# SMLC-NYSBC/TARGET-VAE

Hardware: AMD Instinct MI355X
Metric: training images/sec (fwd+bwd+Adam), P8 z=2 64x64 bs=256/GPU (higher is better)
Workload: dtype f32 (matrix products: operands as TWO fp16 parts under one power-of-two scale PER ROW of the operand (row / column of the product), 3 fp16 MFMAs per product block -- 2 where one operand is the exact 0 / 1 matrix -- fp32 accumulate: at least as accurate against fp64 as the fp32 matrix pipe (profiles/

## Files before the change

target-vae_amd/csrc/dense_wgrad_x6_instance.hip:

```cpp
#include "abi_dense_x6.hpp"

using namespace tvae;

#define TVAE_WG_ONE(V_, X_, L_, NP_)                                                                                  \
    do {                                                                                                              \
        hipError_t e_ = allow_big_lds(dense_wgrad_x6_dma_kernel<V_, X_, L_, NP_>, WG_RING_BYTES);                     \
        if (e_ != hipSuccess) return (int)e_;                                                                         \
        hipLaunchKernelGGL((dense_wgrad_x6_dma_kernel<V_, X_, L_, NP_>), dim3(tm.grid()), dim3(DX6_THREADS),           \
                           WG_RING_BYTES, st, dY, ldd, X, ldx, ws, M, Kf, N, nchunk, tm, bt, dy_stride, vg, va, atile, hs); \
        return (int)hipGetLastError();                                                                                \
    } while (0)
#define TVAE_WG_LAUNCH_DEF(NP_)                                                                                       \
    namespace tvae {                                                                                                  \
    int dense_wgrad_x6_launch_p##NP_(TVAE_WG_LAUNCH_ARGS) {                                                           \
        switch (variant) {                                                                                            \
            case 0: TVAE_WG_ONE(false, false, 0, NP_);                                                            \
            case 1: TVAE_WG_ONE(true, false, 0, NP_);                                                             \
            case 2: TVAE_WG_ONE(false, true, 0, NP_);                                                             \
            case 3: TVAE_WG_ONE(true, true, 0, NP_);                                                              \
            case 5: TVAE_WG_ONE(true, false, 1, NP_);                                                                 \
            case 7: TVAE_WG_ONE(true, true, 1, NP_);                                                                  \
            case 9: TVAE_WG_ONE(true, false, 2, NP_);                                                                 \
            case 11: TVAE_WG_ONE(true, true, 2, NP_);                                                                 \
            default: return (int)hipErrorInvalidValue;                                                                \
        }                                                                                                             \
    }                                                                                                                 \
    }

#define TVAE_WG_LAUNCH_DEF_ABF                                                                                        \
    namespace tvae {                                                                                                  \
    int dense_wgrad_x6_launch_p1_abf(TVAE_WG_LAUNCH_ARGS) {                                                           \
        if (variant != 0) return (int)hipErrorInvalidValue;                                                           \
        hipError_t e_ = allow_big_lds(dense_wgrad_x6_dma_kernel<false, false, 0, 1, true>, WG_RING_BYTES);            \
        if (e_ != hipSuccess) return (int)e_;                                                                         \
        hipLaunchKernelGGL((dense_wgrad_x6_dma_kernel<false, false, 0, 1, true>), dim3(tm.grid()), dim3(DX6_THREADS),  \
                           WG_RING_BYTES, st, dY, ldd, X, ldx, ws, M, Kf, N, nchunk, tm, bt, dy_stride, vg, va, atile, hs); \
        return (int)hipGetLastError();                                                                                \
    }                                                                                                                 \
    }

#define TVAE_WGW_LAUNCH_DEF(NP_)                                                                                      \
    namespace tvae {                                                                                                  \
    int dense_wgrad_x6_wide_p##NP_(TVAE_WGW_LAUNCH_ARGS) {                                                            \
        if (M % WW_ROWS != 0 || Kf <= 128 || bt.tiles_per_batch <= 0 ||                                             \
            tm.tilesN != (Kf <= 160 ? 1 : cdiv(Kf, 192)))                                                             \
            return (int)hipErrorInvalidValue;                                                                         \
        const unsigned grid_ =                                                                                        \
            8u * cdiv(tm.splits * (tm.tilesM / bt.tiles_per_batch), 8) * bt.tiles_per_batch * tm.tilesN;              \
        if (Kf <= 160) {              \
            hipError_t e_ = allow_big_lds(dense_wgrad_x6_wide_kernel<NP_, 5>, WW_RING_BYTES);                         \
            if (e_ != hipSuccess) return (int)e_;                                                                     \
            hipLaunchKernelGGL((dense_wgrad_x6_wide_kernel<NP_, 5>), dim3(grid_), dim3(DX6_THREADS), WW_RING_BYTES, st, \
                               dY, ldd, X, ldx, ws, M, Kf, N, nchunk, tm, bt, dy_stride, atile, hs);                  \
            return (int)hipGetLastError();                                                                            \
        }                                                                                                             \
        hipError_t e_ = allow_big_lds(dense_wgrad_x6_wide_kernel<NP_, 6>, WW_RING_BYTES);                             \
        if (e_ != hipSuccess) return (int)e_;                                                                         \
        hipLaunchKernelGGL((dense_wgrad_x6_wide_kernel<NP_, 6>), dim3(grid_), dim3(DX6_THREADS), WW_RING_BYTES, st,   \
                           dY, ldd, X, ldx, ws, M, Kf, N, nchunk, tm, bt, dy_stride, atile, hs);                      \
        return (int)hipGetLastError();                                                                                \
    }                                                                                                                 \
    }

#if TVAE_WG_NP == 1
TVAE_WG_LAUNCH_DEF(1)
TVAE_WG_LAUNCH_DEF_ABF
#elif TVAE_WG_NP == 2
TVAE_WG_LAUNCH_DEF(2)
TVAE_WGW_LAUNCH_DEF(2)
#elif TVAE_WG_NP == 3
TVAE_WG_LAUNCH_DEF(3)
TVAE_WGW_LAUNCH_DEF(3)
#else
#error "dense_wgrad_x6_instance.hip is compiled once per number of parts: -DTVAE_WG_NP=1, 2 or 3"
#endif
```

target-vae_amd/csrc/dense_x6_kernels.hpp:

```cpp
#pragma once
#include <hip/hip_runtime.h>
#include <type_traits>
#include "conv_x6_device.hpp"
#include "small_device.hpp"

#ifndef TVAE_ABL
#define TVAE_ABL 0
#endif

namespace tvae {

template <int NP>
__device__ __forceinline__ void mfma_np(f32x16& acc, const Cell16 (&a)[3], const Cell16 (&b)[3]) {
    if (NP == 3) mfma6(acc, a, b);
    else if (NP == 2) mfma3h(acc, a, b);
    else acc = __builtin_amdgcn_mfma_f32_32x32x16_bf16(a[0].v, b[0].v, acc, 0, 0, 0);
}
template <int NP>
__device__ __forceinline__ void mfma_part(f32x16& acc, const Cell16& a, const Cell16& b) {
    if (NP == 2) acc = __builtin_amdgcn_mfma_f32_32x32x16_f16(a.h, b.h, acc, 0, 0, 0);
    else acc = __builtin_amdgcn_mfma_f32_32x32x16_bf16(a.v, b.v, acc, 0, 0, 0);
}
template <int NP> struct OneBits { static constexpr unsigned lo = NP == 2 ? 0x3c00u : 0x3f80u, hi = lo << 16; };
template <bool XS>
// ... 753 lines not shown
    if (!tm.decode(blockIdx.x, tile_m, tile_n, split_unused)) return;
    int batch = 0;
    if (bt.tiles_per_batch > 0) {
        batch = tile_m / bt.tiles_per_batch;
        X += batch * bt.x_stride;
        ep.C += batch * bt.c_stride;
    }
    const int m0g = tile_m * DX4_ROWS;
    const int m0 = m0g - batch * bt.tiles_per_batch * DX4_ROWS, n0 = tile_n * 128;
    const int khalf = lane >> 5;
    const int nk = K8pad >> 1;
    bsm[tid] = (ep.bias && (m0 + tid) < M) ? ep.bias[(m0 + tid) >> ep.bias_shift] : 0.f;
    __shared__ __attribute__((aligned(16))) float h3a_[NP == 2 ? DX4_ROWS : 4];
    __shared__ float h3x_[NP == 2 ? 128 : 1];
    float sx = 1.f;
    if (NP == 2) {
        h3a_[tid] = h3_inv(h3_scale(hs.amax_a[hs.a_rows ? m0g + tid : 0]));
        if (hs.x_group > 0) sx = h3_scale(hs.amax_x[(long)batch * hs.x_bstride + min((n0 + (tid & 127)) / hs.x_group, hs.x_bstride - 1)]);
        else sx = h3_scale(hs.amax_x[0]);
        if (tid < 128) h3x_[tid] = h3_inv(sx);
    }

    const long part_cells = (long)K8pad * Mpad;
    const uint4* a_ptr = A3 + (long)khalf * Mpad + m0g + 64 * wave + (lane & 31);
    auto load_a = [&](int t, Cell16 (&a)[2][3]) {
        const uint4* q = a_ptr + (long)(2 * t) * Mpad;
#pragma unroll
        for (int i = 0; i < 2; ++i)
#pragma unroll
            for (int p = 0; p < NP; ++p) a[i][p].u = q[p * part_cells + i * 32];
    };
    const int kq = tid >> 7, nb = tid & 127;
    const float* x_col = X + n0 + nb;
    auto load_x = [&](int t, float (&x)[2][4]) {
#pragma unroll
        for (int h = 0; h < 2; ++h) {
            const int kb = 16 * t + 4 * (kq + 2 * h);
#pragma unroll
            for (int j = 0; j < 4; ++j) x[h][j] = x_col[(long)min(kb + j, K - 1) * ldx];
        }
    };
    auto store_b = [&](int stage, const float (&x)[2][4]) {
#pragma unroll
        for (int h = 0; h < 2; ++h) {
            uint2* dst = reinterpret_cast<uint2*>(Bs + stage * 768 + h * 128 + nb) + kq;
            if (NP == 1) {
                dst[0] = make_uint2(bf16_pair(x[h][0], x[h][1]), bf16_pair(x[h][2], x[h][3]));
                continue;
            }
            if (NP == 2) {
                unsigned hw[2], lw[2];
#pragma unroll
                for (int q = 0; q < 2; ++q) split2h_pair(x[h][2 * q] * sx, x[h][2 * q + 1] * sx, hw[q], lw[q]);
                dst[0] = make_uint2(hw[0], hw[1]);
                dst[2 * 256] = make_uint2(lw[0], lw[1]);
                continue;
            }
            unsigned hw[2], mw[2], lw[2];
#pragma unroll
            for (int q = 0; q < 2; ++q) split3_pair(x[h][2 * q], x[h][2 * q + 1], hw[q], mw[q], lw[q]);
            dst[0] = make_uint2(hw[0], hw[1]);
            dst[2 * 256] = make_uint2(mw[0], mw[1]);
            dst[2 * 512] = make_uint2(lw[0], lw[1]);
        }
    };
    f32x16 acc[2][4];
#pragma unroll
    for (int i = 0; i < 2; ++i)
#pragma unroll
        for (int j = 0; j < 4; ++j)
#pragma unroll
            for (int r = 0; r < 16; ++r) acc[i][j][r] = 0.f;
    Cell16 afA[2][3], afB[2][3];
    float xA[2][4], xB[2][4];
    {
        float x0[2][4];
        load_x(0, x0);
        load_a(0, afA);
        load_x(nk > 1 ? 1 : 0, xB);
        load_x(nk > 2 ? 2 : 0, xA);
        store_b(0, x0);
    }
    __syncthreads();
    auto step = [&](int t, Cell16 (&afc)[2][3], Cell16 (&afn)[2][3], float (&xn)[2][4]) {
        const int cur = t & 1;
        load_a(t + 1 < nk ? t + 1 : t, afn);
        const uint4* bs = Bs + cur * 768 + khalf * 128 + (lane & 31);
#pragma unroll
        for (int j = 0; j < 4; ++j) {
            Cell16 bf[3];
#pragma unroll
            for (int p = 0; p < NP; ++p) bf[p].u = bs[p * 256 + j * 32];
            mfma_np<NP>(acc[0][j], afc[0], bf);
            mfma_np<NP>(acc[1][j], afc[1], bf);
            if (j == 1) {
                store_b(cur ^ 1, xn);
                load_x(t + 3 < nk ? t + 3 : t, xn);
            }
        }
        __builtin_amdgcn_sched_barrier(0);
        __syncthreads();
    };
    int tt = 0;
    for (; tt + 1 < nk; tt += 2) {
        step(tt, afA, afB, xB);
        step(tt + 1, afB, afA, xA);
    }
    if (nk & 1) step(nk - 1, afA, afB, xB);
    if (EPI == 1) {
        if (m0 < M) dense_x6_epilogue_store<NP>(acc, ep.C, ep.ldc, (long)tile_n * ep.ctile, h3a_, h3x_, wave, lane, m0);
        return;
    }
    if (EPI == 2) {
        unsigned short* c16 = reinterpret_cast<unsigned short*>(ep.C - (long)batch * bt.c_stride) + (long)batch * bt.c_stride;
        if (m0 < M) dense_x6_epilogue_store_bf16(acc, c16, ep.ldc, (long)tile_n * ep.ctile, wave, lane, m0);
        return;
    }
    if (NP == 2) h3_unscale_rc<true>(acc, h3a_, h3x_, wave, lane);
    float ysum[4] = {0.f, 0.f, 0.f, 0.f};
    float gsum[4][2] = {{0.f, 0.f}, {0.f, 0.f}, {0.f, 0.f}, {0.f, 0.f}};
    const float gyv[4] = {0.f, 0.f, 0.f, 0.f};
    const InTail it{nullptr, nullptr, nullptr, nullptr, nullptr, nullptr, 1};
    float vmax_ = 0.f;
    if (TVAE_ABL & 8) {
        float t_ = 0.f;
#pragma unroll
        for (int i = 0; i < 2; ++i)
#pragma unroll
            for (int j = 0; j < 4; ++j)
#pragma unroll
                for (int r = 0; r < 16; ++r) t_ += acc[i][j][r];
        if (t_ == 123.456f) ep.C[0] = t_;
    } else
    if (ep.act == ACT_LRELU)
        dense_x6_epilogue<ACT_LRELU, ACT_NONE, false, false, false>(acc, ep, bsm, m0, n0, M, wave, lane, nullptr, ysum, it, nullptr,
                                                                     gsum, tile_n, nullptr, gyv, 0.f, nullptr, 0, vmax_);
    else if (ep.act == ACT_TANH)
        dense_x6_epilogue<ACT_TANH, ACT_NONE, false, false, false>(acc, ep, bsm, m0, n0, M, wave, lane, nullptr, ysum, it, nullptr,
                                                                    gsum, tile_n, nullptr, gyv, 0.f, nullptr, 0, vmax_);
    else
        dense_x6_epilogue<ACT_NONE, ACT_NONE, false, false, false>(acc, ep, bsm, m0, n0, M, wave, lane, nullptr, ysum, it, nullptr,
                                                                    gsum, tile_n, nullptr, gyv, 0.f, nullptr, 0, vmax_);
}

struct ATile {
    int sh;
    int mask;
    long ts;
};
constexpr ATile ATILE_PLAIN = {30, 0x3fffffff, 0};

constexpr int WG_SLOT_BYTES = 4096 + 1024 + 256;
constexpr int WG_RING_BYTES = 8 * 3 * WG_SLOT_BYTES;

template <bool VIRT, bool XVA, int LRF, int NP, bool ABF = false>
static __global__ __launch_bounds__(DX6_THREADS, 2)
void dense_wgrad_x6_dma_kernel(const float* __restrict__ dY, long ldd, const float* __restrict__ X, long ldx, float* ws,
                               int M, int Kf, int N, int nchunk, TileMap tm, DenseBatch bt, long dy_stride, VirtGrad vg,
                               VirtAct va, ATile atile, H3Scale hs) {
    static_assert(!ABF || (NP == 1 && !VIRT && !XVA && LRF == 0), "bf16-stored A: one-part mode, plain operands");
    constexpr int NDMA = (ABF ? 2 : (LRF == 2 ? 2 : 4)) + (XVA ? 2 : 1) + (VIRT ? 1 : 0);
    __shared__ __attribute__((aligned(16))) uint4 Bs[2 * 3 * 2 * 128];
    extern __shared__ __attribute__((aligned(16))) unsigned char wg_ring[];
    const int tid = threadIdx.x, lane = tid & 63;
    const int wave = __builtin_amdgcn_readfirstlane(tid >> 6);
    int tile_m, tile_k, split;
    if (!tm.decode(blockIdx.x, tile_m, tile_k, split)) return;
    int batch = 0, nbatch = 1;
    if (bt.tiles_per_batch > 0) {
        batch = tile_m / bt.tiles_per_batch;
        nbatch = tm.tilesM / bt.tiles_per_batch;
        tile_m -= batch * bt.tiles_per_batch;
        dY += (ABF ? batch * dy_stride / 2 : batch * dy_stride);
        X += batch * bt.x_stride;
    }
    const int m0 = tile_m * DX6_ROWS, k0 = tile_k * 128;
    const int nbeg = split * nchunk;
    const int nend = min(N, nbeg + nchunk);
    const int nk = (nend - nbeg) >> 4;
    const int khalf = lane >> 5;
    if (nk <= 0) {
#pragma unroll
        for (int i = 0; i < 2; ++i)
#pragma unroll
            for (int r = 0; r < 16; ++r) {
                const int m = m0 + wave * 64 + i * 32 + (r & 3) + 8 * (r >> 2) + 4 * khalf;
                if (m >= M) continue;
                float* wrow = ws + (((long)split * nbatch + batch) * M + m) * Kf + k0 + (lane & 31);
#pragma unroll
                for (int j = 0; j < 4; ++j)
                    if (k0 + j * 32 + (lane & 31) < Kf) wrow[j * 32] = 0.f;
            }
        return;
    }

    auto a_scale_of = [&](int m) -> float {
        return h3_scale(hs.amax_a[hs.a_rows ? (long)batch * hs.a_bstride + (hs.a_mod > 0 ? m % hs.a_mod : m) : 0]);
    };
    float sa[2] = {1.f, 1.f};
    if (NP == 2 && !LRF) {
#pragma unroll
        for (int i = 0; i < 2; ++i) sa[i] = a_scale_of(min(m0 + 64 * wave + 32 * i + (lane & 31), M - 1));
    }
    const float* d_ptr[4];
#pragma unroll
    for (int g = 0; g < 4; ++g) {
        if (ABF) {
            const int row = m0 + 64 * wave + 32 * (g & 1) + (lane & 31);
            d_ptr[g] = reinterpret_cast<const float*>(reinterpret_cast<const unsigned short*>(dY) +
                                                      (long)min(row, M - 1) * ldd + 8 * (lane >> 5));
        } else {
            const int row = m0 + 64 * wave + 16 * g + (lane >> 2);
            d_ptr[g] = dY + (long)min(row, M - 1) * ldd + 4 * ((lane & 3) ^ ((lane >> 4) & 3));
        }
    }
    const unsigned* b_ptr[2] = {nullptr, nullptr};
    if (LRF == 2) {
#pragma unroll
        for (int i = 0; i < 2; ++i)
            b_ptr[i] = vg.bits + (long)min(m0 + 64 * wave + 32 * i + (lane & 31), M - 1) * (N >> 5);
    }
    const int kr = tid >> 2, q4 = tid & 3;
    const int kx = min(k0 + kr, Kf - 1);
    const float b_ok = (k0 + kr) < Kf ? 1.f : 0.f;
    const float* x_src = XVA ? va.xr + 2 * (long)nbeg + (lane & 31) : X + (long)kx * ldx + nbeg + 4 * q4;
    const float* lb_src = XVA ? (va.lb ? va.lb + kx : va.bc + kx) : nullptr;
    const float lb_on = (XVA && va.lb) ? 1.f : 0.f;
    const float* g_src = VIRT ? vg.gy + nbeg + (lane & 15) : nullptr;
    const float va_w0 = XVA ? va.wc[2 * kx] : 0.f, va_w1 = XVA ? va.wc[2 * kx + 1] : 0.f, va_bc = XVA ? va.bc[kx] : 0.f;
    float sx = 1.f;
    if (NP == 2) {
        if (XVA && LRF) sx = h3_scale(__fmaf_rn(fabsf(va_w0) + fabsf(va_w1), hs.amax_x[0], hs.amax_x[4 + kx]) * hs.amax_x[3]);
        else if (hs.x_group > 0) sx = h3_scale(hs.amax_x[(long)batch * hs.x_bstride + kx / hs.x_group]);
        else sx = h3_scale(hs.amax_x[0]);
    }
    const unsigned ring_lds = (unsigned)(size_t)(__attribute__((address_space(3))) void*)wg_ring +
                              (unsigned)(wave * 3 * WG_SLOT_BYTES);
    const unsigned char* ring = wg_ring + wave * 3 * WG_SLOT_BYTES;
    auto dma_step = [&](int slot, int t) {
        const int na = nbeg + 16 * t;
        const long off = (long)(na >> atile.sh) * atile.ts + (na & atile.mask);
        const unsigned sl = ring_lds + (unsigned)(slot * WG_SLOT_BYTES);
        if (ABF) {
#pragma unroll
            for (int g = 0; g < 2; ++g) {
                const unsigned short* src = reinterpret_cast<const unsigned short*>(d_ptr[g]) + off;
                const unsigned dst = sl + (unsigned)(g * 1024);
                asm volatile("s_mov_b32 m0, %0\n\ts_nop 0\n\tglobal_load_lds_dwordx4 %1, off" :: "s"(dst), "v"(src) : "memory", "m0");
            }
        } else if (LRF == 2) {
#pragma unroll
            for (int i = 0; i < 2; ++i) {
                const unsigned* src = b_ptr[i] + (na >> 5);
                const unsigned dst = sl + (unsigned)(i * 256);
                asm volatile("s_mov_b32 m0, %0\n\ts_nop 0\n\tglobal_load_lds_dword %1, off" :: "s"(dst), "v"(src) : "memory", "m0");
            }
        } else {
#pragma unroll
            for (int g = 0; g < 4; ++g) {
                const float* src = d_ptr[g] + off;
                const unsigned dst = sl + (unsigned)(g * 1024);
                asm volatile("s_mov_b32 m0, %0\n\ts_nop 0\n\tglobal_load_lds_dwordx4 %1, off" :: "s"(dst), "v"(src) : "memory", "m0");
            }
        }
        if (XVA) {
            const float* sx = x_src + 32 * t;
            const unsigned dx = sl + 4096u;
            asm volatile("s_mov_b32 m0, %0\n\ts_nop 0\n\tglobal_load_lds_dword %1, off" :: "s"(dx), "v"(sx) : "memory", "m0");
            const float* slb = lb_src + (long)(lb_on != 0.f ? na / va.Np : 0) * Kf;
            const unsigned dl = sl + 4096u + 256u;
            asm volatile("s_mov_b32 m0, %0\n\ts_nop 0\n\tglobal_load_lds_dword %1, off" :: "s"(dl), "v"(slb) : "memory", "m0");
        } else {
            const float* sx = x_src + 16 * t;
            const unsigned dx = sl + 4096u;
            asm volatile("s_mov_b32 m0, %0\n\ts_nop 0\n\tglobal_load_lds_dwordx4 %1, off" :: "s"(dx), "v"(sx) : "memory", "m0");
        }
        if (VIRT) {
            const float* sg = g_src + 16 * t;
            const unsigned dg = sl + 4096u + 1024u;
            asm volatile("s_mov_b32 m0, %0\n\ts_nop 0\n\tglobal_load_lds_dword %1, off" :: "s"(dg), "v"(sg) : "memory", "m0");
        }
    };
    int a_at[2][2];
#pragma unroll
    for (int i = 0; i < 2; ++i)
#pragma unroll
        for (int h = 0; h < 2; ++h)
            a_at[i][h] = (2 * i + ((lane >> 4) & 1)) * 1024 + (lane & 15) * 64 + (((2 * khalf + h) ^ ((lane >> 2) & 3)) * 16);
    auto read_a = [&](int slot, float4 (&r)[2][2], float4 (&gq)[2]) {
        const unsigned char* sl = ring + slot * WG_SLOT_BYTES;
        if (ABF) {
#pragma unroll
            for (int i = 0; i < 2; ++i) r[i][0] = *reinterpret_cast<const float4*>(sl + i * 1024 + 16 * lane);
            return;
        }
        if (LRF == 2) {
#pragma unroll
            for (int i = 0; i < 2; ++i) r[i][0].x = *reinterpret_cast<const float*>(sl + i * 256 + 4 * lane);
            return;
        }
#pragma unroll
        for (int i = 0; i < 2; ++i)
#pragma unroll
            for (int h = 0; h < 2; ++h) r[i][h] = *reinterpret_cast<const float4*>(sl + a_at[i][h]);
        if (VIRT && !LRF) {
            gq[0] = *reinterpret_cast<const float4*>(sl + 4096 + 1024 + 32 * khalf);
            gq[1] = *reinterpret_cast<const float4*>(sl + 4096 + 1024 + 32 * khalf + 16);
        }
    };
    const bool xva_lrelu = XVA && va.act == ACT_LRELU;
    auto read_x = [&](int slot) -> float4 {
        const unsigned char* sl = ring + slot * WG_SLOT_BYTES + 4096;
        if (XVA) {
            const float4 c0 = *reinterpret_cast<const float4*>(sl + 32 * q4);
            const float4 c1 = *reinterpret_cast<const float4*>(sl + 32 * q4 + 16);
            const float lbv = *reinterpret_cast<const float*>(sl + 256 + 4 * lane) * lb_on;
            if (xva_lrelu) {
                const float p0 = dec_l0_pre(va_w0, va_w1, va_bc, lbv, c0.x, c0.y), p1 = dec_l0_pre(va_w0, va_w1, va_bc, lbv, c0.z, c0.w);
                const float p2 = dec_l0_pre(va_w0, va_w1, va_bc, lbv, c1.x, c1.y), p3 = dec_l0_pre(va_w0, va_w1, va_bc, lbv, c1.z, c1.w);
                if (va.slope > 0.f && va.slope < 1.f)
                    return make_float4(fmaxf(p0, p0 * va.slope), fmaxf(p1, p1 * va.slope), fmaxf(p2, p2 * va.slope),
                                       fmaxf(p3, p3 * va.slope));
                return make_float4(p0 > 0.f ? p0 : p0 * va.slope, p1 > 0.f ? p1 : p1 * va.slope, p2 > 0.f ? p2 : p2 * va.slope,
                                   p3 > 0.f ? p3 : p3 * va.slope);
            }
            return make_float4(act_apply(dec_l0_pre(va_w0, va_w1, va_bc, lbv, c0.x, c0.y), va.act, va.slope),
                               act_apply(dec_l0_pre(va_w0, va_w1, va_bc, lbv, c0.z, c0.w), va.act, va.slope),
                               act_apply(dec_l0_pre(va_w0, va_w1, va_bc, lbv, c1.x, c1.y), va.act, va.slope),
                               act_apply(dec_l0_pre(va_w0, va_w1, va_bc, lbv, c1.z, c1.w), va.act, va.slope));
        }
        return *reinterpret_cast<const float4*>(sl + 16 * lane);
    };
    float a_ok[2];
#pragma unroll
    for (int i = 0; i < 2; ++i) {
        const int m = m0 + 64 * wave + 32 * i + (lane & 31);
        a_ok[i] = m < M ? ((VIRT && !LRF) ? vg.wo[m] : 1.f) : 0.f;
    }
    auto virt_a = [&](float4 (&r)[2][2], const float4 (&gq)[2]) {
        if (VIRT && !LRF) {
#pragma unroll
            for (int i = 0; i < 2; ++i)
#pragma unroll
                for (int h = 0; h < 2; ++h)
                    r[i][h] = make_float4(virt_value(vg, r[i][h].x, 1.f, gq[h].x), virt_value(vg, r[i][h].y, 1.f, gq[h].y),
                                          virt_value(vg, r[i][h].z, 1.f, gq[h].z), virt_value(vg, r[i][h].w, 1.f, gq[h].w));
        }
    };
    auto split_a = [&](const float4 (&r)[2][2], Cell16 (&a)[2][3], int t) {
        if (ABF) {
#pragma unroll
            for (int i = 0; i < 2; ++i)
                a[i][0].u = make_uint4(__float_as_uint(r[i][0].x), __float_as_uint(r[i][0].y), __float_as_uint(r[i][0].z),
                                       __float_as_uint(r[i][0].w));
            return;
        }
        if (LRF == 2) {
            const int sh = ((nbeg + 16 * t) & 31) + 8 * khalf;
#pragma unroll
            for (int i = 0; i < 2; ++i) {
                const unsigned b = (__float_as_uint(r[i][0].x) >> sh) & 0xffu;
                const unsigned y = b | (b << 15);
#pragma unroll
                for (int q = 0; q < 4; ++q) a[i][0].w[q] = (y & (0x00010001u << (2 * q))) * (OneBits<NP>::lo >> (2 * q));
            }
            return;
        }
        if (LRF) {
#pragma unroll
            for (int i = 0; i < 2; ++i) {
                const float v[8] = {r[i][0].x, r[i][0].y, r[i][0].z, r[i][0].w, r[i][1].x, r[i][1].y, r[i][1].z, r[i][1].w};
#pragma unroll
                for (int q = 0; q < 4; ++q)
                    a[i][0].w[q] = (v[2 * q] > 0.f ? OneBits<NP>::lo : 0u) | (v[2 * q + 1] > 0.f ? OneBits<NP>::hi : 0u);
            }
            return;
        }
#pragma unroll
        for (int i = 0; i < 2; ++i) {
            const float f = NP == 2 ? a_ok[i] * sa[i] : a_ok[i];
            const float v[8] = {r[i][0].x * f, r[i][0].y * f, r[i][0].z * f, r[i][0].w * f,
                                r[i][1].x * f, r[i][1].y * f, r[i][1].z * f, r[i][1].w * f};
            if (NP == 1) {
#pragma unroll
                for (int q = 0; q < 4; ++q) a[i][0].w[q] = bf16_pair(v[2 * q], v[2 * q + 1]);
            } else if (NP == 2) {
                split2hx8(v, a[i][0], a[i][1]);
            } else {
                split3x8(v, a[i][0], a[i][1], a[i][2]);
            }
        }
    };
    float ssum = 0.f;
    const float bsx = NP == 2 ? b_ok * sx : b_ok;
    auto store_b = [&](int stage, const float4& x, int slot, bool real_step) {
        unsigned hw[2], mw[2], lw[2];
        float4 gm = make_float4(bsx, bsx, bsx, bsx);
        if (LRF) {
            const float4 g4 = *reinterpret_cast<const float4*>(ring + slot * WG_SLOT_BYTES + 4096 + 1024 + 16 * q4);
            gm = make_float4(g4.x * bsx, g4.y * bsx, g4.z * bsx, g4.w * bsx);
        }
        const float v[4] = {x.x * gm.x, x.y * gm.y, x.z * gm.z, x.w * gm.w};
        if (LRF && real_step) ssum += (v[0] + v[1]) + (v[2] + v[3]);
        uint2* dst = reinterpret_cast<uint2*>(Bs + stage * 768 + (q4 >> 1) * 128 + kr) + (q4 & 1);
        if (NP == 1) {
            dst[0] = make_uint2(bf16_pair(v[0], v[1]), bf16_pair(v[2], v[3]));
            return;
        }
        if (NP == 2) {
#pragma unroll
            for (int q = 0; q < 2; ++q) split2h_pair(v[2 * q], v[2 * q + 1], hw[q], lw[q]);
            dst[0] = make_uint2(hw[0], hw[1]);
            dst[2 * 256] = make_uint2(lw[0], lw[1]);
            return;
        }
#pragma unroll
        for (int q = 0; q < 2; ++q) split3_pair(v[2 * q], v[2 * q + 1], hw[q], mw[q], lw[q]);
        dst[0] = make_uint2(hw[0], hw[1]);
        dst[2 * 256] = make_uint2(mw[0], mw[1]);
        dst[2 * 512] = make_uint2(lw[0], lw[1]);
    };

    f32x16 acc[2][4];
#pragma unroll
    for (int i = 0; i < 2; ++i)
#pragma unroll
        for (int j = 0; j < 4; ++j)
#pragma unroll
            for (int r = 0; r < 16; ++r) acc[i][j][r] = 0.f;

    Cell16 af[2][3];
    const int tl = nk - 1;
    {
        dma_step(0, 0);
        dma_step(1, min(1, tl));
        dma_step(2, min(2, tl));
        asm volatile("s_waitcnt vmcnt(%0)" :: "n"(2 * NDMA) : "memory");
        float4 ar[2][2], g0[2];
        read_a(0, ar, g0);
        virt_a(ar, g0);
        split_a(ar, af, 0);
        store_b(0, read_x(0), 0, true);
    }
    __syncthreads();
    int s_next = 1, s_dma = 0;
    for (int t = 0; t < nk; ++t) {
        const int cur = t & 1;
        asm volatile("s_waitcnt vmcnt(%0)" :: "n"(NDMA) : "memory");
        dma_step(s_dma, min(t + 3, tl));
        Cell16 an[2][3];
        const uint4* bs = Bs + cur * 768 + khalf * 128 + (lane & 31);
#pragma unroll
        for (int j = 0; j < 4; ++j) {
            Cell16 bf[3];
#pragma unroll
            for (int p = 0; p < NP; ++p) bf[p].u = bs[p * 256 + j * 32];
            if (LRF) {
#pragma unroll
                for (int i = 0; i < 2; ++i)
#pragma unroll
                    for (int p = 0; p < NP; ++p) mfma_part<NP>(acc[i][j], af[i][0], bf[p]);
            } else {
                mfma_np<NP>(acc[0][j], af[0], bf);
                mfma_np<NP>(acc[1][j], af[1], bf);
            }
            if (j == 0) {
                float4 ar[2][2], gn[2];
                read_a(s_next, ar, gn);
                virt_a(ar, gn);
                split_a(ar, an, min(t + 1, tl));
            }
            if (j == 1) store_b(cur ^ 1, read_x(s_next), s_next, t + 1 < nk);
        }
#pragma unroll
        for (int i = 0; i < 2; ++i)
#pragma unroll
            for (int p = 0; p < 3; ++p) af[i][p] = an[i][p];
        s_next = s_next == 2 ? 0 : s_next + 1;
        s_dma = s_dma == 2 ? 0 : s_dma + 1;
        __builtin_amdgcn_sched_barrier(0);
        __syncthreads();
    }
    asm volatile("s_waitcnt vmcnt(0)" ::: "memory");
    float sk[4] = {0.f, 0.f, 0.f, 0.f};
    float ixv[4] = {1.f, 1.f, 1.f, 1.f};
    float* ssm = reinterpret_cast<float*>(Bs);
    if (LRF) {
        ssum += __shfl_xor(ssum, 1, 64);
        ssum += __shfl_xor(ssum, 2, 64);
        if (q4 == 0) ssm[kr] = NP == 2 ? ssum * h3_inv(sx) : ssum;
    }
    if (NP == 2) {
        if (q4 == 0) ssm[128 + kr] = h3_inv(sx);
        if (!LRF) ssm[256 + tid] = h3_inv(a_scale_of(min(m0 + tid, M - 1)));
    }
    if (LRF || NP == 2) __syncthreads();
    if (LRF) {
#pragma unroll
        for (int j = 0; j < 4; ++j) sk[j] = vg.slope * ssm[j * 32 + (lane & 31)];
    }
    if (NP == 2) {
#pragma unroll
        for (int j = 0; j < 4; ++j) ixv[j] = ssm[128 + j * 32 + (lane & 31)];
    }
    const float oms = 1.f - vg.slope;
    if (TVAE_ABL & 8) {
        float t_ = 0.f;
#pragma unroll
        for (int i = 0; i < 2; ++i)
#pragma unroll
            for (int j = 0; j < 4; ++j)
#pragma unroll
                for (int r = 0; r < 16; ++r) t_ += acc[i][j][r];
        if (t_ == 123.456f) ws[0] = t_;
        return;
    }
#pragma unroll
    for (int i = 0; i < 2; ++i)
#pragma unroll
        for (int r = 0; r < 16; ++r) {
            const int rl = wave * 64 + i * 32 + (r & 3) + 8 * (r >> 2) + 4 * (lane >> 5);
            const int m = m0 + rl;
            if (m >= M) continue;
            const float wm = (LRF && !vg.raw) ? vg.wo[m] : 1.f;
            const float ia = (NP == 2 && !LRF) ? ssm[256 + rl] : 1.f;
            float* wrow = ws + (((long)split * nbatch + batch) * M + m) * Kf + k0 + (lane & 31);
#pragma unroll
            for (int j = 0; j < 4; ++j)
                if (k0 + j * 32 + (lane & 31) < Kf) {
                    const float a = NP == 2 ? (acc[i][j][r] * ia) * ixv[j] : acc[i][j][r];
                    wrow[j * 32] = LRF ? wm * __fmaf_rn(oms, a, sk[j]) : a;
                }
        }
}

template <int NP, int NK>
static __global__ __launch_bounds__(256, 1)
void dense_x6_xres_kernel(const uint4* __restrict__ A3, const float* __restrict__ X, long ldx, float* __restrict__ C, long ldc,
                           long ctile, int M, int Mb, int Mpad, int K, int nprob, int tilesN, int nch, long x_stride,
                           long c_stride, H3Scale hs) {
    extern __shared__ __attribute__((aligned(16))) unsigned char xres_lds[];
    const int tid = threadIdx.x, lane = tid & 63;
    const int wave = __builtin_amdgcn_readfirstlane(tid >> 6);
    constexpr int K8pad = 2 * NK;
    uint4* Bs = reinterpret_cast<uint4*>(xres_lds);
    float* h3a_ = reinterpret_cast<float*>(xres_lds + (size_t)NK * NP * 256 * 16);
    float* h3x_ = h3a_ + Mb;
    const int cs = (tilesN + nch - 1) / nch;
    const int g = ((blockIdx.x >> 3) / cs) * 8 + (blockIdx.x & 7), r = (blockIdx.x >> 3) % cs;
    const int batch = g / nch, tile_n = (g - batch * nch) * cs + r;
    if (batch >= nprob || tile_n >= tilesN) return;
    X += batch * x_stride;
    C += batch * c_stride + (long)tile_n * ctile;
    const int n0 = tile_n * 128;
    const int khalf = lane >> 5;
    {
        const int kq = tid >> 7, nb = tid & 127;
        float sx = 1.f;
        if (NP == 2) {
            sx = hs.x_group > 0 ? h3_scale(hs.amax_x[(long)batch * hs.x_bstride + min((n0 + nb) / hs.x_group, hs.x_bstride - 1)])
                                : h3_scale(hs.amax_x[0]);
            if (tid < 128) h3x_[tid] = h3_inv(sx);
            for (int m = tid; m < Mb; m += 256) h3a_[m] = h3_inv(h3_scale(hs.amax_a[hs.a_rows ? batch * Mb + m : 0]));
        }
        const float* x_col = X + n0 + nb;
#pragma unroll
        for (int t0 = 0; t0 < NK; t0 += 3) {
            float x[3][2][4];
#pragma unroll
            for (int u = 0; u < 3; ++u)
#pragma unroll
                for (int h = 0; h < 2; ++h)
#pragma unroll
                    for (int j = 0; j < 4; ++j) {
                        const int k = 16 * (t0 + u < NK ? t0 + u : NK - 1) + 4 * (kq + 2 * h) + j;
                        x[u][h][j] = x_col[(long)min(k, K - 1) * ldx];
                    }
#pragma unroll
            for (int u = 0; u < 3; ++u) {
                if (t0 + u >= NK) break;
#pragma unroll
                for (int h = 0; h < 2; ++h) {
                    uint2* dst = reinterpret_cast<uint2*>(Bs + (size_t)(t0 + u) * NP * 256 + h * 128 + nb) + kq;
                    if (NP == 2) {
                        unsigned hw[2], lw[2];
#pragma unroll
                        for (int q = 0; q < 2; ++q) split2h_pair(x[u][h][2 * q] * sx, x[u][h][2 * q + 1] * sx, hw[q], lw[q]);
                        dst[0] = make_uint2(hw[0], hw[1]);
                        dst[2 * 256] = make_uint2(lw[0], lw[1]);
                    } else {
                        unsigned hw[2], mw[2], lw[2];
#pragma unroll
                        for (int q = 0; q < 2; ++q) split3_pair(x[u][h][2 * q], x[u][h][2 * q + 1], hw[q], mw[q], lw[q]);
                        dst[0] = make_uint2(hw[0], hw[1]);
                        dst[2 * 256] = make_uint2(mw[0], mw[1]);
                        dst[2 * 512] = make_uint2(lw[0], lw[1]);
                    }
                }
            }
        }
    }
    __syncthreads();
    const long part_cells = (long)K8pad * Mpad;
    const uint4* bs0 = Bs + khalf * 128 + (lane & 31);
    const uint4* a_base = A3 + (long)khalf * Mpad + (long)batch * Mb + (lane & 31);
    float ixv[4];
#pragma unroll
    for (int j = 0; j < 4; ++j) ixv[j] = NP == 2 ? h3x_[j * 32 + (lane & 31)] : 1.f;
    const unsigned loff = (unsigned)((4 * khalf * ldc + (lane & 31)) * 4);
    auto store_row = [&](const f32x16 (&acc)[2][4], int mp, int s_) {
        const int i = s_ >> 4, q = (s_ >> 2) & 3, p = s_ & 3;
        const int row = mp + 32 * i + 8 * q + p;
        float* rowp = reinterpret_cast<float*>(reinterpret_cast<char*>(C + (long)row * ldc) + loff);
        const float ia = NP == 2 ? h3a_[row + 4 * khalf] : 1.f;
#pragma unroll
        for (int j = 0; j < 4; ++j) {
            const float v = NP == 2 ? (acc[i][j][4 * q + p] * ixv[j]) * ia : acc[i][j][4 * q + p];
            __builtin_nontemporal_store(v, rowp + j * 32);
        }
    };
    auto block = [&](f32x16 (&accC)[2][4], int mc, const f32x16 (&accP)[2][4], int mp, bool have_prev) {
        const uint4* a_run[NP];
#pragma unroll
        for (int p = 0; p < NP; ++p) a_run[p] = a_base + mc + p * part_cells;
#ifndef TVAE_XRES2_NB
#define TVAE_XRES2_NB 8
#endif
        constexpr int NB = TVAE_XRES2_NB;
        Cell16 af[NB][2][3];
        auto load_next = [&](Cell16 (&a)[2][3]) {
#pragma unroll
            for (int p = 0; p < NP; ++p) {
                a[0][p].u = a_run[p][0];
                a[1][p].u = a_run[p][32];
// ... 264 lines not shown
```

Before: 26840.

## Process 32-column steps in sign-bit wgrad kernel with recomputed operand

```diff
diff --git a/target-vae_amd/csrc/dense_wgrad_x6_instance.hip b/target-vae_amd/csrc/dense_wgrad_x6_instance.hip
--- a/target-vae_amd/csrc/dense_wgrad_x6_instance.hip
+++ b/target-vae_amd/csrc/dense_wgrad_x6_instance.hip
@@ -2,6 +2,25 @@
 
 using namespace tvae;
 
+#ifdef TVAE_WG_STEP16
+constexpr bool WG_STEP32 = false;
+#else
+constexpr bool WG_STEP32 = true;
+#endif
+#define TVAE_WG_BITS_XVA(NP_)                                                                                         \
+    do {                                                                                                              \
+        if constexpr (WG_STEP32) {                                                                                    \
+            if (nchunk % 32 == 0 && N % 32 == 0 && va.Np >= 32 && va.Np % 32 == 0) {                                  \
+                hipError_t e_ = allow_big_lds(dense_wgrad_x6_dma_kernel<true, true, 2, NP_, false, 32>, WG32_RING_BYTES); \
+                if (e_ != hipSuccess) return (int)e_;                                                                 \
+                hipLaunchKernelGGL((dense_wgrad_x6_dma_kernel<true, true, 2, NP_, false, 32>), dim3(tm.grid()),       \
+                                   dim3(DX6_THREADS), WG32_RING_BYTES, st, dY, ldd, X, ldx, ws, M, Kf, N, nchunk, tm, bt, \
+                                   dy_stride, vg, va, atile, hs);                                                     \
+                return (int)hipGetLastError();                                                                        \
+            }                                                                                                         \
+        }                                                                                                             \
+        TVAE_WG_ONE(true, true, 2, NP_);                                                                              \
+    } while (0)
 #define TVAE_WG_ONE(V_, X_, L_, NP_)                                                                                  \
     do {                                                                                                              \
         hipError_t e_ = allow_big_lds(dense_wgrad_x6_dma_kernel<V_, X_, L_, NP_>, WG_RING_BYTES);                     \
@@ -21,7 +40,7 @@
             case 5: TVAE_WG_ONE(true, false, 1, NP_);                                                                 \
             case 7: TVAE_WG_ONE(true, true, 1, NP_);                                                                  \
             case 9: TVAE_WG_ONE(true, false, 2, NP_);                                                                 \
-            case 11: TVAE_WG_ONE(true, true, 2, NP_);                                                                 \
+            case 11: TVAE_WG_BITS_XVA(NP_);                                                                           \
             default: return (int)hipErrorInvalidValue;                                                                \
         }                                                                                                             \
     }                                                                                                                 \
diff --git a/target-vae_amd/csrc/dense_x6_kernels.hpp b/target-vae_amd/csrc/dense_x6_kernels.hpp
--- a/target-vae_amd/csrc/dense_x6_kernels.hpp
+++ b/target-vae_amd/csrc/dense_x6_kernels.hpp
@@ -929,15 +929,21 @@
 
 constexpr int WG_SLOT_BYTES = 4096 + 1024 + 256;
 constexpr int WG_RING_BYTES = 8 * 3 * WG_SLOT_BYTES;
-
-template <bool VIRT, bool XVA, int LRF, int NP, bool ABF = false>
+constexpr int WG32_SLOT_BYTES = 5 * 256;
+constexpr int WG32_RING_BYTES = 8 * 3 * WG32_SLOT_BYTES;
+
+template <bool VIRT, bool XVA, int LRF, int NP, bool ABF = false, int STEP = 16>
 static __global__ __launch_bounds__(DX6_THREADS, 2)
 void dense_wgrad_x6_dma_kernel(const float* __restrict__ dY, long ldd, const float* __restrict__ X, long ldx, float* ws,
                                int M, int Kf, int N, int nchunk, TileMap tm, DenseBatch bt, long dy_stride, VirtGrad vg,
                                VirtAct va, ATile atile, H3Scale hs) {
     static_assert(!ABF || (NP == 1 && !VIRT && !XVA && LRF == 0), "bf16-stored A: one-part mode, plain operands");
+    static_assert(STEP == 16 || (STEP == 32 && VIRT && XVA && LRF == 2), "32-column steps: sign bits x recomputed operand");
+    constexpr bool S32 = STEP == 32;
     constexpr int NDMA = (ABF ? 2 : (LRF == 2 ? 2 : 4)) + (XVA ? 2 : 1) + (VIRT ? 1 : 0);
-    __shared__ __attribute__((aligned(16))) uint4 Bs[2 * 3 * 2 * 128];
+    constexpr int SLOT = S32 ? WG32_SLOT_BYTES : WG_SLOT_BYTES, XOFF = S32 ? 512 : 4096, GOFF = S32 ? 1024 : 4096 + 1024;
+    constexpr int BPART = S32 ? 512 : 256, BSTAGE = S32 ? NP * 512 : 768;
+    __shared__ __attribute__((aligned(16))) uint4 Bs[2 * BSTAGE];
     extern __shared__ __attribute__((aligned(16))) unsigned char wg_ring[];
     const int tid = threadIdx.x, lane = tid & 63;
     const int wave = __builtin_amdgcn_readfirstlane(tid >> 6);
@@ -954,7 +960,7 @@
     const int m0 = tile_m * DX6_ROWS, k0 = tile_k * 128;
     const int nbeg = split * nchunk;
     const int nend = min(N, nbeg + nchunk);
-    const int nk = (nend - nbeg) >> 4;
+    const int nk = (nend - nbeg) >> (S32 ? 5 : 4);
     const int khalf = lane >> 5;
     if (nk <= 0) {
 #pragma unroll
@@ -1000,10 +1006,10 @@
     const int kr = tid >> 2, q4 = tid & 3;
     const int kx = min(k0 + kr, Kf - 1);
     const float b_ok = (k0 + kr) < Kf ? 1.f : 0.f;
-    const float* x_src = XVA ? va.xr + 2 * (long)nbeg + (lane & 31) : X + (long)kx * ldx + nbeg + 4 * q4;
+    const float* x_src = XVA ? va.xr + 2 * (long)nbeg + (S32 ? lane : lane & 31) : X + (long)kx * ldx + nbeg + 4 * q4;
     const float* lb_src = XVA ? (va.lb ? va.lb + kx : va.bc + kx) : nullptr;
     const float lb_on = (XVA && va.lb) ? 1.f : 0.f;
-    const float* g_src = VIRT ? vg.gy + nbeg + (lane & 15) : nullptr;
+    const float* g_src = VIRT ? vg.gy + nbeg + (lane & (STEP - 1)) : nullptr;
     const float va_w0 = XVA ? va.wc[2 * kx] : 0.f, va_w1 = XVA ? va.wc[2 * kx + 1] : 0.f, va_bc = XVA ? va.bc[kx] : 0.f;
     float sx = 1.f;
     if (NP == 2) {
@@ -1012,12 +1018,13 @@
         else sx = h3_scale(hs.amax_x[0]);
     }
     const unsigned ring_lds = (unsigned)(size_t)(__attribute__((address_space(3))) void*)wg_ring +
-                              (unsigned)(wave * 3 * WG_SLOT_BYTES);
-    const unsigned char* ring = wg_ring + wave * 3 * WG_SLOT_BYTES;
+                              (unsigned)(wave * 3 * SLOT);
+    const unsigned char* ring = wg_ring + wave * 3 * SLOT;
+    int img = S32 ? nbeg / va.Np : 0, img_end = S32 ? (img + 1) * va.Np : 0;
     auto dma_step = [&](int slot, int t) {
-        const int na = nbeg + 16 * t;
+        const int na = nbeg + STEP * t;
         const long off = (long)(na >> atile.sh) * atile.ts + (na & atile.mask);
-        const unsigned sl = ring_lds + (unsigned)(slot * WG_SLOT_BYTES);
+        const unsigned sl = ring_lds + (unsigned)(slot * SLOT);
         if (ABF) {
 #pragma unroll
             for (int g = 0; g < 2; ++g) {
@@ -1041,11 +1048,15 @@
             }
         }
         if (XVA) {
-            const float* sx = x_src + 32 * t;
-            const unsigned dx = sl + 4096u;
+            const float* sx = x_src + 2 * STEP * t;
+            const unsigned dx = sl + (unsigned)XOFF;
             asm volatile("s_mov_b32 m0, %0\n\ts_nop 0\n\tglobal_load_lds_dword %1, off" :: "s"(dx), "v"(sx) : "memory", "m0");
-            const float* slb = lb_src + (long)(lb_on != 0.f ? na / va.Np : 0) * Kf;
-            const unsigned dl = sl + 4096u + 256u;
+            if (S32 && na >= img_end) {
+                ++img;
+                img_end += va.Np;
+            }
+            const float* slb = lb_src + (long)(lb_on != 0.f ? (S32 ? img : na / va.Np) : 0) * Kf;
+            const unsigned dl = sl + (unsigned)XOFF + 256u;
             asm volatile("s_mov_b32 m0, %0\n\ts_nop 0\n\tglobal_load_lds_dword %1, off" :: "s"(dl), "v"(slb) : "memory", "m0");
         } else {
             const float* sx = x_src + 16 * t;
@@ -1053,8 +1064,8 @@
             asm volatile("s_mov_b32 m0, %0\n\ts_nop 0\n\tglobal_load_lds_dwordx4 %1, off" :: "s"(dx), "v"(sx) : "memory", "m0");
         }
         if (VIRT) {
-            const float* sg = g_src + 16 * t;
-            const unsigned dg = sl + 4096u + 1024u;
+            const float* sg = g_src + STEP * t;
+            const unsigned dg = sl + (unsigned)GOFF;
             asm volatile("s_mov_b32 m0, %0\n\ts_nop 0\n\tglobal_load_lds_dword %1, off" :: "s"(dg), "v"(sg) : "memory", "m0");
         }
     };
@@ -1065,7 +1076,7 @@
         for (int h = 0; h < 2; ++h)
             a_at[i][h] = (2 * i + ((lane >> 4) & 1)) * 1024 + (lane & 15) * 64 + (((2 * khalf + h) ^ ((lane >> 2) & 3)) * 16);
     auto read_a = [&](int slot, float4 (&r)[2][2], float4 (&gq)[2]) {
-        const unsigned char* sl = ring + slot * WG_SLOT_BYTES;
+        const unsigned char* sl = ring + slot * SLOT;
         if (ABF) {
 #pragma unroll
             for (int i = 0; i < 2; ++i) r[i][0] = *reinterpret_cast<const float4*>(sl + i * 1024 + 16 * lane);
@@ -1086,11 +1097,11 @@
         }
     };
     const bool xva_lrelu = XVA && va.act == ACT_LRELU;
-    auto read_x = [&](int slot) -> float4 {
-        const unsigned char* sl = ring + slot * WG_SLOT_BYTES + 4096;
+    auto read_x = [&](int slot, int half = 0) -> float4 {
+        const unsigned char* sl = ring + slot * SLOT + XOFF;
         if (XVA) {
-            const float4 c0 = *reinterpret_cast<const float4*>(sl + 32 * q4);
-            const float4 c1 = *reinterpret_cast<const float4*>(sl + 32 * q4 + 16);
+            const float4 c0 = *reinterpret_cast<const float4*>(sl + 128 * half + 32 * q4);
+            const float4 c1 = *reinterpret_cast<const float4*>(sl + 128 * half + 32 * q4 + 16);
             const float lbv = *reinterpret_cast<const float*>(sl + 256 + 4 * lane) * lb_on;
             if (xva_lrelu) {
                 const float p0 = dec_l0_pre(va_w0, va_w1, va_bc, lbv, c0.x, c0.y), p1 = dec_l0_pre(va_w0, va_w1, va_bc, lbv, c0.z, c0.w);
@@ -1170,16 +1181,19 @@
     };
     float ssum = 0.f;
     const float bsx = NP == 2 ? b_ok * sx : b_ok;
-    auto store_b = [&](int stage, const float4& x, int slot, bool real_step) {
+    auto store_b = [&](int stage, const float4& x, int slot, bool real_step, int half = 0) {
         unsigned hw[2], mw[2], lw[2];
         float4 gm = make_float4(bsx, bsx, bsx, bsx);
         if (LRF) {
-            const float4 g4 = *reinterpret_cast<const float4*>(ring + slot * WG_SLOT_BYTES + 4096 + 1024 + 16 * q4);
+            const float4 g4 = *reinterpret_cast<const float4*>(ring + slot * SLOT + GOFF + 64 * half + 16 * q4);
             gm = make_float4(g4.x * bsx, g4.y * bsx, g4.z * bsx, g4.w * bsx);
         }
         const float v[4] = {x.x * gm.x, x.y * gm.y, x.z * gm.z, x.w * gm.w};
-        if (LRF && real_step) ssum += (v[0] + v[1]) + (v[2] + v[3]);
-        uint2* dst = reinterpret_cast<uint2*>(Bs + stage * 768 + (q4 >> 1) * 128 + kr) + (q4 & 1);
+        if (LRF && real_step) {
+            if (S32) ssum += __fmaf_rn(x.x, gm.x, v[1]) + __fmaf_rn(x.z, gm.z, v[3]);
+            else ssum += (v[0] + v[1]) + (v[2] + v[3]);
+        }
+        uint2* dst = reinterpret_cast<uint2*>(Bs + stage * BSTAGE + (2 * half + (q4 >> 1)) * 128 + kr) + (q4 & 1);
         if (NP == 1) {
             dst[0] = make_uint2(bf16_pair(v[0], v[1]), bf16_pair(v[2], v[3]));
             return;
@@ -1188,14 +1202,14 @@
 #pragma unroll
             for (int q = 0; q < 2; ++q) split2h_pair(v[2 * q], v[2 * q + 1], hw[q], lw[q]);
             dst[0] = make_uint2(hw[0], hw[1]);
-            dst[2 * 256] = make_uint2(lw[0], lw[1]);
+            dst[2 * BPART] = make_uint2(lw[0], lw[1]);
             return;
         }
 #pragma unroll
         for (int q = 0; q < 2; ++q) split3_pair(v[2 * q], v[2 * q + 1], hw[q], mw[q], lw[q]);
         dst[0] = make_uint2(hw[0], hw[1]);
-        dst[2 * 256] = make_uint2(mw[0], mw[1]);
-        dst[2 * 512] = make_uint2(lw[0], lw[1]);
+        dst[2 * BPART] = make_uint2(mw[0], mw[1]);
+        dst[4 * BPART] = make_uint2(lw[0], lw[1]);
     };
 
     f32x16 acc[2][4];
@@ -1206,57 +1220,111 @@
 #pragma unroll
             for (int r = 0; r < 16; ++r) acc[i][j][r] = 0.f;
 
-    Cell16 af[2][3];
     const int tl = nk - 1;
-    {
-        dma_step(0, 0);
-        dma_step(1, min(1, tl));
-        dma_step(2, min(2, tl));
-        asm volatile("s_waitcnt vmcnt(%0)" :: "n"(2 * NDMA) : "memory");
-        float4 ar[2][2], g0[2];
-        read_a(0, ar, g0);
-        virt_a(ar, g0);
-        split_a(ar, af, 0);
-        store_b(0, read_x(0), 0, true);
-    }
-    __syncthreads();
-    int s_next = 1, s_dma = 0;
-    for (int t = 0; t < nk; ++t) {
-        const int cur = t & 1;
-        asm volatile("s_waitcnt vmcnt(%0)" :: "n"(NDMA) : "memory");
-        dma_step(s_dma, min(t + 3, tl));
-        Cell16 an[2][3];
-        const uint4* bs = Bs + cur * 768 + khalf * 128 + (lane & 31);
-#pragma unroll
-        for (int j = 0; j < 4; ++j) {
-            Cell16 bf[3];
-#pragma unroll
-            for (int p = 0; p < NP; ++p) bf[p].u = bs[p * 256 + j * 32];
-            if (LRF) {
-#pragma unroll
-                for (int i = 0; i < 2; ++i)
-#pragma unroll
-                    for (int p = 0; p < NP; ++p) mfma_part<NP>(acc[i][j], af[i][0], bf[p]);
-            } else {
-                mfma_np<NP>(acc[0][j], af[0], bf);
-                mfma_np<NP>(acc[1][j], af[1], bf);
-            }
-            if (j == 0) {
-                float4 ar[2][2], gn[2];
-                read_a(s_next, ar, gn);
-                virt_a(ar, gn);
-                split_a(ar, an, min(t + 1, tl));
-            }
-            if (j == 1) store_b(cur ^ 1, read_x(s_next), s_next, t + 1 < nk);
-        }
-#pragma unroll
-        for (int i = 0; i < 2; ++i)
-#pragma unroll
-            for (int p = 0; p < 3; ++p) af[i][p] = an[i][p];
-        s_next = s_next == 2 ? 0 : s_next + 1;
-        s_dma = s_dma == 2 ? 0 : s_dma + 1;
-        __builtin_amdgcn_sched_barrier(0);
+    if constexpr (S32) {
+        Cell16 afA[2][2][3], afB[2][2][3];
+        {
+            dma_step(0, 0);
+            dma_step(1, min(1, tl));
+            dma_step(2, min(2, tl));
+            asm volatile("s_waitcnt vmcnt(%0)" :: "n"(2 * NDMA) : "memory");
+            float4 ar[2][2], g0[2];
+            read_a(0, ar, g0);
+            split_a(ar, afA[0], 0);
+            split_a(ar, afA[1], 1);
+            store_b(0, read_x(0, 0), 0, true, 0);
+            store_b(0, read_x(0, 1), 0, true, 1);
+        }
         __syncthreads();
+        int s_next = 1, s_dma = 0;
+        auto step = [&](int t, Cell16 (&afc)[2][2][3], Cell16 (&afn)[2][2][3]) {
+            const int cur = t & 1;
+            asm volatile("s_waitcnt vmcnt(%0)" :: "n"(NDMA) : "memory");
+            dma_step(s_dma, min(t + 3, tl));
+#pragma unroll
+            for (int u = 0; u < 2; ++u) {
+                const uint4* bs = Bs + cur * BSTAGE + (2 * u + khalf) * 128 + (lane & 31);
+#pragma unroll
+                for (int j = 0; j < 4; ++j) {
+                    Cell16 bf[3];
+#pragma unroll
+                    for (int p = 0; p < NP; ++p) bf[p].u = bs[p * BPART + j * 32];
+#pragma unroll
+                    for (int i = 0; i < 2; ++i)
+#pragma unroll
+                        for (int p = 0; p < NP; ++p) mfma_part<NP>(acc[i][j], afc[u][i][0], bf[p]);
+                    if (u == 0 && j == 0) {
+                        float4 ar[2][2], gn[2];
+                        read_a(s_next, ar, gn);
+                        split_a(ar, afn[0], 0);
+                        split_a(ar, afn[1], 1);
+                    }
+                    if (j == 1) store_b(cur ^ 1, read_x(s_next, u), s_next, t + 1 < nk, u);
+                }
+            }
+            s_next = s_next == 2 ? 0 : s_next + 1;
+            s_dma = s_dma == 2 ? 0 : s_dma + 1;
+            __builtin_amdgcn_sched_barrier(0);
+            __syncthreads();
+        };
+        int tt = 0;
+        for (; tt + 1 < nk; tt += 2) {
+            step(tt, afA, afB);
+            step(tt + 1, afB, afA);
+        }
+        if (nk & 1) step(nk - 1, afA, afB);
+    } else {
+        Cell16 af[2][3];
+        {
+            dma_step(0, 0);
+            dma_step(1, min(1, tl));
+            dma_step(2, min(2, tl));
+            asm volatile("s_waitcnt vmcnt(%0)" :: "n"(2 * NDMA) : "memory");
+            float4 ar[2][2], g0[2];
+            read_a(0, ar, g0);
+            virt_a(ar, g0);
+            split_a(ar, af, 0);
+            store_b(0, read_x(0), 0, true);
+        }
+        __syncthreads();
+        int s_next = 1, s_dma = 0;
+        for (int t = 0; t < nk; ++t) {
+            const int cur = t & 1;
+            asm volatile("s_waitcnt vmcnt(%0)" :: "n"(NDMA) : "memory");
+            dma_step(s_dma, min(t + 3, tl));
+            Cell16 an[2][3];
+            const uint4* bs = Bs + cur * 768 + khalf * 128 + (lane & 31);
+#pragma unroll
+            for (int j = 0; j < 4; ++j) {
+                Cell16 bf[3];
+#pragma unroll
+                for (int p = 0; p < NP; ++p) bf[p].u = bs[p * 256 + j * 32];
+                if (LRF) {
+#pragma unroll
+                    for (int i = 0; i < 2; ++i)
+#pragma unroll
+                        for (int p = 0; p < NP; ++p) mfma_part<NP>(acc[i][j], af[i][0], bf[p]);
+                } else {
+                    mfma_np<NP>(acc[0][j], af[0], bf);
+                    mfma_np<NP>(acc[1][j], af[1], bf);
+                }
+                if (j == 0) {
+                    float4 ar[2][2], gn[2];
+                    read_a(s_next, ar, gn);
+                    virt_a(ar, gn);
+                    split_a(ar, an, min(t + 1, tl));
+                }
+                if (j == 1) store_b(cur ^ 1, read_x(s_next), s_next, t + 1 < nk);
+            }
+#pragma unroll
+            for (int i = 0; i < 2; ++i)
+#pragma unroll
+                for (int p = 0; p < 3; ++p) af[i][p] = an[i][p];
+            s_next = s_next == 2 ? 0 : s_next + 1;
+            s_dma = s_dma == 2 ? 0 : s_dma + 1;
+            __builtin_amdgcn_sched_barrier(0);
+            __syncthreads();
+        }
     }
     asm volatile("s_waitcnt vmcnt(0)" ::: "memory");
     float sk[4] = {0.f, 0.f, 0.f, 0.f};
```

After: 27520, median of 6. 1.03x the previous value.
